# Algy/fast-slic

Hardware: AMD Instinct MI355X
Metric: megapixels/sec @10 iters (1280x720 & 4K, K=1600); % HBM roofline (higher is better)
Workload: dtype u8/u16/i32 (integer SLIC); 1 GPU; 1280x720 RGB, K=1600, 10 iters (configs[1]), 8 frames/GPU; frames_per_gpu=8, global_frames=8, slots_per_gpu=6, submissions_per_launch_group=up to 2 (dynamic batching of the pipeline), inputs=device-resident uint8 RGB, device int16 labels, parallelism=frames sharded across GPUs, no collective

## Files before the change

### fast_slic_amd/csrc/assign.hip

```cpp
#include "device_common.h"
#include <type_traits>

namespace fslic {



template <int R, bool FUSE, bool LUT>
__global__ __launch_bounds__(256) void k_assign(FrameDev f, int rem, int stride, int Hv, int buf, int sbuf) {
    extern __shared__ uint32_t s_lut[];
    __shared__ uint32_t s_rawbuf[kWavesPerBlock][3 * 64];
    __shared__ uint4 s_listbuf[kWavesPerBlock][64];
    __shared__ uint32_t s_accbuf[FUSE ? kWavesPerBlock * kAccSlots * 6 * kAccCopies : 1];

    f.select(blockIdx.z);
    const uint32_t gen = f.generation();
    const int tid = threadIdx.x;
    const int lane = tid & 63;
    const int wave = (int)rfl((uint32_t)(tid >> 6));
    uint32_t* const s_raw = s_rawbuf[wave];
    uint4* const s_list = s_listbuf[wave];
    uint32_t* const s_acc = s_accbuf + (FUSE ? wave * (kAccSlots * 6 * kAccCopies) : 0);
    const int W = f.W, S = f.S;
    const int x0 = blockIdx.x * kTileW;
    const int x = x0 + lane;
// ... 118 lines not shown
        };
        for (int c0 = 0; c0 < total; c0 += 64) {
            const int e = c0 + lane;
            ClusterRec rec;
            rec.yx = 0; rec.lab = 0; rec.tag = 0; rec.pad = 0;
            if (e < total) rec = citems[cell_slot(e)];
            stream(rec, e < total && rec.pad == gen && in_window(rec, win));
        }
        for (uint32_t i0 = 0; i0 < novf; i0 += 64) {
            const uint32_t i = i0 + lane;
            ClusterRec rec;
            rec.yx = 0; rec.lab = 0; rec.tag = 0; rec.pad = 0;
            if (i < novf) rec = oitems[i];
            stream(rec, i < novf && in_window(rec, win));
        }
#pragma unroll
        for (int r = 0; r < R; ++r) {
            if (!(okx && r < nrows)) continue;
            const int y = yw_lo + r * stride;
            const size_t p = (size_t)y * W + x;
            uint32_t lbl;
            if (bw[r] < kHuge) { lbl = bt[r] & 0xFFFFu; f.labels[p] = (uint16_t)lbl; }
            else if (f.first_visit(y)) { lbl = 0xFFFFu; f.labels[p] = (uint16_t)0xFFFFu; }
            else lbl = f.labels[p];
            if (FUSE && lbl != 0xFFFFu) global_accumulate(f.sums[0], lbl, (uint32_t)y, (uint32_t)x, pix[r]);
        }
        return;
    }

    int n;
    {
        const bool act = lane < nraw;
        const uint32_t yx_j = act ? s_raw[lane] : 0u;
        const uint32_t lab_j = act ? s_raw[64 + lane] : 0u;
        const uint32_t tag_j = act ? s_raw[128 + lane] : 0xFFFFFFFFu;
        bool dup = false;
        for (int i = 0; i < nraw; ++i) {
            const uint32_t ty = __builtin_amdgcn_readlane(yx_j, i);
            const uint32_t tl = __builtin_amdgcn_readlane(lab_j, i);
            const uint32_t tt = __builtin_amdgcn_readlane(tag_j, i);
            dup = dup || (act && (tt < tag_j) && (ty == yx_j) && (tl == lab_j));
        }
        const unsigned long long dupmask = __ballot(dup);
        int rank = 0;
        for (int i = 0; i < nraw; ++i) {
            const uint32_t tt = __builtin_amdgcn_readlane(tag_j, i);
            rank += (int)((((dupmask >> i) & 1ull) == 0ull) && tt < tag_j);
        }
        if (act && !dup) s_list[rank] = make_uint4(yx_j, lab_j, tag_j & 0xFFFFu, 0u);
        n = nraw - __popcll(dupmask);
    }
    __builtin_amdgcn_wave_barrier();

    uint32_t best[R];
#pragma unroll
    for (int r = 0; r < R; ++r) best[r] = 0xFFFFFFFFu;
    uint2 nxt = *reinterpret_cast<const uint2*>(&s_list[0]);
#pragma unroll 1
    for (int c = 0; c < n; ++c) {
        const uint2 rec = nxt;
        nxt = *reinterpret_cast<const uint2*>(&s_list[min(c + 1, 63)]);
        const uint32_t cyx = rfl(rec.x);
        const uint32_t clab = rfl(rec.y);
        const int cy = (int)(cyx >> 16), cx = (int)(cyx & 0xFFFFu);
        const uint32_t A = spatial_A(cx);
#pragma unroll
        for (int r = 0; r < R; ++r) {
            const uint32_t w = dist_w(r, cy, clab, A);
            best[r] = min(best[r], LUT ? (w | (uint32_t)c) : ((w & hi16) | (uint32_t)c));
        }
    }

    uint32_t slot[R];
#pragma unroll
    for (int r = 0; r < R; ++r) {
        const int y = yw_lo + r * stride;
        const bool ok = okx && r < nrows;
        const bool found = best[r] < kHuge;
        const uint32_t idx = found ? (best[r] & 0xFFFFu) : 0u;
        const uint32_t k = s_list[idx].z;
        slot[r] = 0xFFFFFFFFu;
        if (ok) {
            const size_t p = (size_t)y * W + x;
            if (found) {
                f.labels[p] = (uint16_t)k;
                if (FUSE) {
                    if (idx < (uint32_t)kAccSlots) slot[r] = idx;
                    else global_accumulate(f.sums[0], k, (uint32_t)y, (uint32_t)x, pix[r]);
                }
            } else if (f.first_visit(y)) {
                f.labels[p] = (uint16_t)0xFFFFu;
            } else if (FUSE) {
                const uint32_t old = f.labels[p];
                if (old != 0xFFFFu) global_accumulate(f.sums[0], old, (uint32_t)y, (uint32_t)x, pix[r]);
            }
        }
    }
    if (FUSE) {
        bool uni = slot[0] != 0xFFFFFFFFu;
#pragma unroll
        for (int r = 1; r < R; ++r) uni = uni && (slot[r] == slot[0]);
        const uint32_t copy = (uint32_t)lane & (kAccCopies - 1);
        if (uni) {
            uint32_t sL = 0, sa = 0, sb = 0;
#pragma unroll
            for (int r = 0; r < R; ++r) { sL += pix[r] & 255u; sa += (pix[r] >> 8) & 255u; sb += (pix[r] >> 16) & 255u; }
            uint32_t* a = s_acc + (slot[0] * 6) * kAccCopies + copy;
            atomicAdd(a + 0 * kAccCopies, (uint32_t)R);
            atomicAdd(a + 1 * kAccCopies, (uint32_t)(R * yw_lo + stride * (R * (R - 1) / 2)));
            atomicAdd(a + 2 * kAccCopies, (uint32_t)(R * x));
            atomicAdd(a + 3 * kAccCopies, sL);
            atomicAdd(a + 4 * kAccCopies, sa);
            atomicAdd(a + 5 * kAccCopies, sb);
        } else {
#pragma unroll
            for (int r = 0; r < R; ++r) {
                if (slot[r] != 0xFFFFFFFFu) {
                    uint32_t* a = s_acc + (slot[r] * 6) * kAccCopies + copy;
                    atomicAdd(a + 0 * kAccCopies, 1u);
                    atomicAdd(a + 1 * kAccCopies, (uint32_t)(yw_lo + r * stride));
                    atomicAdd(a + 2 * kAccCopies, (uint32_t)x);
                    atomicAdd(a + 3 * kAccCopies, pix[r] & 255u);
                    atomicAdd(a + 4 * kAccCopies, (pix[r] >> 8) & 255u);
                    atomicAdd(a + 5 * kAccCopies, (pix[r] >> 16) & 255u);
                }
            }
        }
        __builtin_amdgcn_wave_barrier();
        const int nacc = min(n, kAccSlots) * 6;
        for (int i = lane; i < nacc; i += 64) {
            uint32_t v = 0;
#pragma unroll
            for (int c = 0; c < kAccCopies; ++c) v += s_acc[i * kAccCopies + c];
            if (v) {
                const int sl = i / 6;
                atomicAdd(f.sums[0] + 6 * (size_t)s_list[sl].z + (i - sl * 6), v);
            }
        }
    }
}

typedef unsigned short us2 __attribute__((ext_vector_type(2)));

constexpr uint32_t kNoSlot = 0xFFFFFFFFu;
constexpr int kRawBuffer = 0x00020000;
constexpr int kAuxSc1 = 16;

static __device__ __forceinline__ us2 key_pair(uint32_t dist01, uint32_t idx01) {
    uint32_t r;
    asm("v_pk_mad_u16 %0, %1, 64, %2 op_sel_hi:[1,0,1] clamp" : "=v"(r) : "v"(dist01), "s"(idx01));
    return __builtin_bit_cast(us2, r);
}


static __device__ __forceinline__ unsigned long long sbitrep(uint32_t v) {
    unsigned long long r;
    asm("s_bitreplicate_b64_b32 %0, %1" : "=s"(r) : "s"(v));
    return r;
}
static __device__ __forceinline__ void min_in_place(us2& best, us2 key) {
    uint32_t b = __builtin_bit_cast(uint32_t, best);
    asm("v_pk_min_u16 %0, %0, %1" : "+v"(b) : "v"(__builtin_bit_cast(uint32_t, key)));
    best = __builtin_bit_cast(us2, b);
}

template <int R>
static __device__ __forceinline__ void row_masks(uint32_t inv, uint32_t (&m)[R / 2]) {
    static_assert(R == 8 || R == 16 || R == 32, "row masks are built for 8, 16 or 32 rows");
    if constexpr (R == 32) {
        uint32_t lo[8], hi[8];
        row_masks<16>(inv & 0xFFFFu, lo);
        row_masks<16>(inv >> 16, hi);
#pragma unroll
        for (int q = 0; q < 8; ++q) { m[q] = lo[q]; m[8 + q] = hi[q]; }
        return;
    }
    const unsigned long long r1 = sbitrep(inv);
    const unsigned long long r2 = sbitrep((uint32_t)r1);
    if (R == 8) {
        const unsigned long long r3 = sbitrep((uint32_t)r2);
        const unsigned long long a = sbitrep((uint32_t)r3), b = sbitrep((uint32_t)(r3 >> 32));
        m[0] = (uint32_t)a; m[1] = (uint32_t)(a >> 32); m[2] = (uint32_t)b; m[3] = (uint32_t)(b >> 32);
    } else {
        const unsigned long long r3a = sbitrep((uint32_t)r2), r3b = sbitrep((uint32_t)(r2 >> 32));
        const unsigned long long q0 = sbitrep((uint32_t)r3a), q1 = sbitrep((uint32_t)(r3a >> 32));
        const unsigned long long q2 = sbitrep((uint32_t)r3b), q3 = sbitrep((uint32_t)(r3b >> 32));
        m[0] = (uint32_t)q0; m[1] = (uint32_t)(q0 >> 32); m[2] = (uint32_t)q1; m[3] = (uint32_t)(q1 >> 32);
        m[R / 2 - 4] = (uint32_t)q2; m[R / 2 - 3] = (uint32_t)(q2 >> 32); m[R / 2 - 2] = (uint32_t)q3; m[R / 2 - 1] = (uint32_t)(q3 >> 32);
    }
}

#if defined(FSLIC_LAB) && FSLIC_LAB == 4
#define ASG_STAMP(i_, cond_) do { if ((cond_) && lane == 0) { asm volatile("" ::: "memory"); asg_w[(i_)] = (uint32_t)__builtin_amdgcn_s_memrealtime() - asg_t0; asm volatile("" ::: "memory"); } } while (0)
#define ASG_PUT(i_, cond_, v_) do { if ((cond_) && lane == 0) asg_w[(i_)] = (uint32_t)(v_); } while (0)
#else
#define ASG_STAMP(i_, cond_) do { } while (0)
#define ASG_PUT(i_, cond_, v_) do { } while (0)
#endif
#ifdef FSLIC_MARKS
#define ASG_MARK(name_) asm volatile("; @@MARK " name_ ::: "memory")
#else
#define ASG_MARK(name_) do { } while (0)
#endif
static __device__ __forceinline__ void lds_dma_16(const void* gsrc, uint32_t lds_byte_addr) {
    uint32_t keep;
    asm volatile("s_mov_b32 %0, m0\n\ts_mov_b32 m0, %2\n\ts_nop 0\n\tglobal_load_lds_dwordx4 %1, off\n\ts_mov_b32 m0, %0"
                 : "=&s"(keep) : "v"(gsrc), "s"(lds_byte_addr) : "memory");
}

static __device__ __forceinline__ uint32_t ld_agent(const uint32_t* p) { return __hip_atomic_load(p, __ATOMIC_RELAXED, __HIP_MEMORY_SCOPE_AGENT); }
static __device__ __forceinline__ unsigned long long ld_agent64(const void* p) {
    return __hip_atomic_load(reinterpret_cast<const unsigned long long*>(p), __ATOMIC_RELAXED, __HIP_MEMORY_SCOPE_AGENT);
}
static __device__ __forceinline__ void bin_insert_next(const FrameDev& f, uint32_t k, uint32_t yx, uint32_t lab) {
    const int y = (int)(yx >> 16), x = (int)(yx & 0xFFFFu);
    const uint32_t phase = 2u * (div_by((uint32_t)y, (uint32_t)f.T, f.T_rcp) & 1u) + (div_by((uint32_t)x, (uint32_t)f.T, f.T_rcp) & 1u);
    ClusterRec rec;
    rec.yx = yx; rec.lab = lab; rec.tag = (phase << 16) | k; rec.pad = f.generation() + 1u;
    f.cl_tag[k] = rec.tag;
    const int cell = (y >> f.cs_shift) * f.ncx + (x >> f.cs_shift);
    const uint32_t slot = atomicAdd(&f.cell_cnt[1][cell], 1u);
    if (slot < (uint32_t)kCellCap) f.cell_items[1][(size_t)cell * kCellCap + slot] = rec;
    else f.ovf_items[1][atomicAdd(f.ovf_cnt[1], 1u)] = rec;
}
static __device__ __forceinline__ void fused_finalize(const FrameDev& f, uint32_t k, uint32_t yx, uint32_t lab, uint32_t nx, uint32_t ny, uint32_t b0, uint32_t ymask) {
    uint32_t* const s0 = f.sums[0] + 6 * (size_t)k;
    uint32_t s[6];
#pragma unroll
    for (int q = 0; q < 6; ++q) s[q] = ld_agent(s0 + q);
    const char* const cp = reinterpret_cast<const char*>(f.cpart + (size_t)k * f.cpart_ns * 6);
    const uint32_t ne = nx * ny;
    const uint32_t inv_nx = (uint32_t)(65536.0f * __builtin_amdgcn_rcpf((float)nx)) + 1u;
    constexpr int kBatch = 4;
    for (uint32_t e0 = 0; e0 < ne; e0 += kBatch) {
        unsigned long long v[kBatch][3];
#pragma unroll
        for (int u = 0; u < kBatch; ++u) {
            const uint32_t e = e0 + (uint32_t)u;
            uint32_t ey = __umul24(e, inv_nx) >> 16;
            if (__umul24(ey, nx) > e) ey--;
            const uint32_t ex = e - __umul24(ey, nx);
            v[u][0] = v[u][1] = v[u][2] = 0ull;
            if (e < ne) {
                const char* p = cp + __umul24(cpart_slot((b0 >> 16) + ey, (b0 & 0xFFFFu) + ex, ymask, (uint32_t)f.nbx), 24u);
                v[u][0] = ld_agent64(p); v[u][1] = ld_agent64(p + 8); v[u][2] = ld_agent64(p + 16);
            }
        }
#pragma unroll
        for (int u = 0; u < kBatch; ++u) {
            s[0] += (uint32_t)v[u][0]; s[1] += (uint32_t)(v[u][0] >> 32); s[2] += (uint32_t)v[u][1]; s[3] += (uint32_t)(v[u][1] >> 32);
            s[4] += (uint32_t)v[u][2]; s[5] += (uint32_t)(v[u][2] >> 32);
        }
    }
    const uint32_t n = s[0];
    f.cl_n[k] = n;
    if (n != 0) {
        const uint32_t h = n >> 1, r = 0xFFFFFFFFu / n;
        int y = (int)div_by(s[1] + h, n, r), x = (int)div_by(s[2] + h, n, r);
        y = min(max(y, 0), f.H - 1);
        x = min(max(x, 0), f.W - 1);
        const uint32_t L = div_by(s[3] + h, n, r), a = div_by(s[4] + h, n, r), b = div_by(s[5] + h, n, r);
        yx = ((uint32_t)y << 16) | (uint32_t)x;
        lab = (L & 255u) | ((a & 255u) << 8) | ((b & 255u) << 16);
        f.cl_lab[k] = lab;
        f.cl_moved[k] = 1;
        f.cl_yx[k] = yx;
    }
#pragma unroll
    for (int q = 0; q < 6; ++q) s0[q] = 0u;
    f.cl_arrive[k] = 0u;
    bin_insert_next(f, k, yx, lab);
    if (n != 0 && k + 1u < (uint32_t)f.K && f.cl_shadow[k + 1u]) {
        f.cl_shadow[k + 1u] = 0u;
        bin_insert_next(f, k + 1u, f.cl_yx[k + 1u], f.cl_lab[k + 1u]);
    }
}

struct BlkMap { uint32_t gx, gy; };
static inline BlkMap blk_map(dim3 g) { BlkMap m; m.gx = g.x; m.gy = g.y; return m; }
static inline dim3 blk_grid(dim3 g) { return dim3(g.x, g.z, g.y); }

template <int R, bool FUSE, int STRIDE, bool VT, bool FBIN = false, bool PRE = false>
static __device__ __forceinline__ void assign_blk2_body(FrameDev& f, int rem, int Hv, const BlkMap& bm) {
    static_assert(!FBIN || FUSE, "the cluster pass rides on the fused centroid sums");
    static_assert(!PRE || (FUSE && !FBIN), "preemptive mode: the fused pass with its own flush");
    const uint32_t bxi = blockIdx.x, byi = blockIdx.z, bzi = blockIdx.y;
    extern __shared__ __attribute__((aligned(16))) uint32_t s_dyn[];
    __shared__ __attribute__((aligned(16))) uint4 s_raw[kWavesPerBlock][64];
    __shared__ __attribute__((aligned(16))) uint32_t s_part[64][4];
    __shared__ __attribute__((aligned(16))) uint32_t s_wcnt[4];
    __shared__ __attribute__((aligned(16))) uint32_t s_entry[FUSE ? 64 : 4];
    __shared__ __attribute__((aligned(16))) uint16_t s_klab[64];
    __shared__ __attribute__((aligned(16))) unsigned long long s_acc[FUSE ? 64 * kBlkCopies * 2 : 2];
    static_assert(R % 2 == 0, "rows are processed in pairs");
    constexpr int BH = kWavesPerBlock * R;
    static_assert(!FUSE || (BH * 64 * 255 < (1 << 20) && (BH - 1) * STRIDE * BH * 64 < (1 << 20)), "accumulator fields overflow");

    ASG_MARK("entry");
    f.select((int)bzi);
    const uint32_t gen = f.generation();
    const int tid = threadIdx.x;
    if (FBIN) {

        const uint32_t gi = (byi * bm.gx + bxi) * 256u + (uint32_t)tid;
        if (gi < (uint32_t)f.ncell) f.cell_cnt[0][gi] = 0u;
        if (gi == 0u) *f.ovf_cnt[2] = 0u;
// ... 182 lines not shown
        uint32_t va_j, vb_j;
        {
            const int dy0 = yw_lo - (int)(yx_j >> 16);
            const int rs = min(max(div_stride(-dy0 + STRIDE * BIAS + STRIDE - 1) - BIAS, 0), R);
            const int ra = min(max(div_stride(-S - dy0 + STRIDE * BIAS + STRIDE - 1) - BIAS, 0), R);
            const int rb = min(max(div_stride(S - dy0 + STRIDE * BIAS) - BIAS, -1), R - 1);
            const uint32_t upto_rs = low_bits(rs);
            const uint32_t in_win = rb < 0 ? 0u : (low_bits(rb + 1) & ~low_bits(ra) & full);
            va_j = in_win & upto_rs;
            vb_j = in_win & ~upto_rs;
        }
        const uint4* const s_rv = reinterpret_cast<const uint4*>(s_dyn);
        auto pass = [&](uint32_t clab, uint32_t base, uint32_t idx01, const uint32_t* mq) {
            uint32_t spw[R / 2];
            {
                const uint4 e0 = s_rv[base];
                spw[0] = e0.x; spw[1] = e0.y; spw[2] = e0.z; spw[3] = e0.w;
#pragma unroll
                for (int h = 1; h < R / 8; ++h) {
                    const uint4 e1 = s_rv[base + 8 * h * STRIDE];
                    spw[4 * h] = e1.x; spw[4 * h + 1] = e1.y; spw[4 * h + 2] = e1.z; spw[4 * h + 3] = e1.w;
                }
            }
            uint32_t t[R / 2];
#pragma unroll
            for (int q = 0; q < R / 2; ++q) {
                const uint32_t s0 = __builtin_amdgcn_sad_u8(pix[2 * q], clab, spw[q]);
                t[q] = __builtin_amdgcn_sad_hi_u8(pix[2 * q + 1], clab, s0);
            }
            us2 key[R / 2];
#pragma unroll
            for (int q = 0; q < R / 2; ++q) key[q] = key_pair(t[q], mq ? (mq[q] | idx01) : idx01);
#pragma unroll
            for (int q = 0; q < R / 2; ++q) min_in_place(best[q], key[q]);
        };
        unsigned long long todo_wa = todo & ballot(va_j == full);
        unsigned long long todo_wb = todo & ballot(vb_j == full);
        unsigned long long todo_above = todo & ballot(va_j != 0u) & ~todo_wa;
        unsigned long long todo_below = todo & ballot(vb_j != 0u) & ~todo_wb;
        auto fetch = [&](int c, uint32_t& clab, uint32_t& uxc, uint32_t& k0, uint32_t& idx01, auto clamp_tag) {
            constexpr bool CLAMP = decltype(clamp_tag)::value;
            const uint32_t cyx = __builtin_amdgcn_readlane(yx_j, c);
            const uint32_t clabx = __builtin_amdgcn_readlane(lab_j, c);
            clab = clabx & 0x00FFFFFFu;
            const int cy = (int)(cyx >> 16), cx = (int)(cyx & 0xFFFFu);
            const uint32_t ux = __builtin_amdgcn_sad_u16((uint32_t)x, (uint32_t)cx, 0u);
            uxc = CLAMP ? (ux <= (uint32_t)S ? ux : xout) : ux;
            k0 = (uint32_t)(Cc + yw_lo - cy);
            idx01 = (clabx >> 24) * 0x10001u;
        };
#pragma unroll 1
        while (todo_wa) {
            const int c = __builtin_ctzll(todo_wa);
            todo_wa &= todo_wa - 1ull;
            uint32_t clab, uxc, k0, idx01;
            fetch(c, clab, uxc, k0, idx01, std::false_type{});
            if (uxc <= (uint32_t)S) pass(clab, k0 - uxc, idx01, nullptr);
        }
#pragma unroll 1
        while (todo_wb) {
            const int c = __builtin_ctzll(todo_wb);
            todo_wb &= todo_wb - 1ull;
            uint32_t clab, uxc, k0, idx01;
            fetch(c, clab, uxc, k0, idx01, std::false_type{});
            if (uxc <= (uint32_t)S) pass(clab, k0 + uxc, idx01, nullptr);
        }
        if constexpr (R == 16 && FUSE) {
            auto pass_half = [&](auto half_tag, uint32_t clab, uint32_t base, uint32_t idx01, const uint32_t* mq4) {
                constexpr int HF = decltype(half_tag)::value;
                const uint4 e0 = s_rv[base + 8 * HF * STRIDE];
                const uint32_t spw[4] = {e0.x, e0.y, e0.z, e0.w};
                uint32_t t[4];
#pragma unroll
                for (int q = 0; q < 4; ++q) {
                    const uint32_t s0 = __builtin_amdgcn_sad_u8(pix[2 * (4 * HF + q)], clab, spw[q]);
                    t[q] = __builtin_amdgcn_sad_hi_u8(pix[2 * (4 * HF + q) + 1], clab, s0);
                }
                us2 key[4];
#pragma unroll
                for (int q = 0; q < 4; ++q) key[q] = key_pair(t[q], mq4[q] | idx01);
#pragma unroll
                for (int q = 0; q < 4; ++q) min_in_place(best[4 * HF + q], key[q]);
            };
            auto masked = [&](unsigned long long m, const uint32_t rows_j, auto sign_tag) {
                constexpr int SG = decltype(sign_tag)::value;
                unsigned long long m_lo = m & ballot((rows_j & 0xFF00u) == 0u);
                unsigned long long m_hi = m & ballot((rows_j & 0x00FFu) == 0u) & ~m_lo;
                unsigned long long m_both = m & ~m_lo & ~m_hi;
#pragma unroll 1
                while (m_lo) {
                    const int c = __builtin_ctzll(m_lo);
                    m_lo &= m_lo - 1ull;
                    uint32_t clab, uxc, k0, idx01, mq[4];
                    fetch(c, clab, uxc, k0, idx01, std::true_type{});
                    row_masks<8>(~__builtin_amdgcn_readlane(rows_j, c) & 0xFFu, mq);
                    pass_half(std::integral_constant<int, 0>{}, clab, SG < 0 ? k0 - uxc : k0 + uxc, idx01, mq);
                }
#pragma unroll 1
                while (m_hi) {
                    const int c = __builtin_ctzll(m_hi);
                    m_hi &= m_hi - 1ull;
                    uint32_t clab, uxc, k0, idx01, mq[4];
                    fetch(c, clab, uxc, k0, idx01, std::true_type{});
                    row_masks<8>(~(__builtin_amdgcn_readlane(rows_j, c) >> 8) & 0xFFu, mq);
                    pass_half(std::integral_constant<int, 1>{}, clab, SG < 0 ? k0 - uxc : k0 + uxc, idx01, mq);
                }
#pragma unroll 1
                while (m_both) {
                    const int c = __builtin_ctzll(m_both);
                    m_both &= m_both - 1ull;
                    uint32_t clab, uxc, k0, idx01, mq[R / 2];
                    fetch(c, clab, uxc, k0, idx01, std::true_type{});
                    row_masks<R>(~__builtin_amdgcn_readlane(rows_j, c) & full, mq);
                    pass(clab, SG < 0 ? k0 - uxc : k0 + uxc, idx01, mq);
                }
            };
            masked(todo_above, va_j, std::integral_constant<int, -1>{});
            masked(todo_below, vb_j, std::integral_constant<int, 1>{});
        } else {
#pragma unroll 1
            while (todo_above) {
                const int c = __builtin_ctzll(todo_above);
                todo_above &= todo_above - 1ull;
                uint32_t clab, uxc, k0, idx01, mq[R / 2];
                fetch(c, clab, uxc, k0, idx01, std::true_type{});
                row_masks<R>(~__builtin_amdgcn_readlane(va_j, c) & full, mq);
                pass(clab, k0 - uxc, idx01, mq);
            }
#pragma unroll 1
            while (todo_below) {
                const int c = __builtin_ctzll(todo_below);
                todo_below &= todo_below - 1ull;
                uint32_t clab, uxc, k0, idx01, mq[R / 2];
                fetch(c, clab, uxc, k0, idx01, std::true_type{});
                row_masks<R>(~__builtin_amdgcn_readlane(vb_j, c) & full, mq);
                pass(clab, k0 + uxc, idx01, mq);
            }
        }
    } else {
        constexpr int HQ = R / 4;
        static_assert(R % 4 == 0, "two halves of whole row pairs");
        unsigned long long todo_b, todo_u, todo_l;
        {
            const int cyj = (int)(yx_j >> 16);
            const int yh = yw_lo + (R / 2) * STRIDE;
            const unsigned long long up = todo & ballot(cyj <= yw_lo + (R / 2 - 1) * STRIDE + S);
            const unsigned long long lo = todo & ballot(cyj >= yh - S) & ballot(cyj <= yh + (R / 2 - 1) * STRIDE + S);
            todo_b = up & lo;
            todo_u = up & ~lo;
            todo_l = lo & ~up;
        }
        uint32_t pitch_v;
        asm volatile("v_mov_b32 %0, %1" : "=v"(pitch_v) : "s"(nrpad * 4u));
        const char* const tab_b = reinterpret_cast<const char*>(s_dyn);
        auto walk = [&](unsigned long long m, auto q0_tag, auto nq_tag) {
            constexpr int Q0 = decltype(q0_tag)::value, NQ = decltype(nq_tag)::value;
#pragma unroll 1
            while (m) {
                const int c = __builtin_ctzll(m);
                m &= m - 1ull;
                const uint32_t cyx = __builtin_amdgcn_readlane(yx_j, c);
                const uint32_t clabx = __builtin_amdgcn_readlane(lab_j, c);
                const uint32_t clab = clabx & 0x00FFFFFFu;
                const int cy = (int)(cyx >> 16), cx = (int)(cyx & 0xFFFFu);
                const uint32_t ux = __builtin_amdgcn_sad_u16((uint32_t)x, (uint32_t)cx, 0u);
                const uint32_t uxc = min(ux, (uint32_t)(S + 1));
                const uint32_t a0 = __umul24(uxc, pitch_v) + (uint32_t)(yw_lo - cy + dyoff) * 4u;
                const uint32_t idx01 = (clabx >> 24) * 0x10001u;
                uint32_t t[NQ];
#pragma unroll
                for (int q = 0; q < NQ; ++q) {
                    const uint32_t sp = *reinterpret_cast<const uint32_t*>(tab_b + a0 + (uint32_t)((2 * (Q0 + q)) * STRIDE * 4));
                    const uint32_t s0 = __builtin_amdgcn_sad_u8(pix[2 * (Q0 + q)], clab, sp);
                    t[q] = __builtin_amdgcn_sad_hi_u8(pix[2 * (Q0 + q) + 1], clab, s0);
                }
                us2 key[NQ];
#pragma unroll
                for (int q = 0; q < NQ; ++q) key[q] = key_pair(t[q], idx01);
#pragma unroll
                for (int q = 0; q < NQ; ++q) min_in_place(best[Q0 + q], key[q]);
            }
        };
        if constexpr (R == 16 && FUSE) {
            (void)todo_b; (void)todo_u; (void)todo_l;
            unsigned long long cov[4];
            {
                const int cyj = (int)(yx_j >> 16);
#pragma unroll
                for (int q = 0; q < 4; ++q) {
                    const int ylo = yw_lo + q * (R / 4) * STRIDE, yhi = ylo + (R / 4 - 1) * STRIDE;
                    cov[q] = todo & ballot(cyj >= ylo - S) & ballot(cyj <= yhi + S);
                }
            }
            constexpr int P = R / 8;
            auto quarters = [&](unsigned long long m, auto q0, auto nq) {
                walk(m, std::integral_constant<int, decltype(q0)::value * P>{}, std::integral_constant<int, decltype(nq)::value * P>{});
            };
            using I0 = std::integral_constant<int, 0>; using I1 = std::integral_constant<int, 1>; using I2 = std::integral_constant<int, 2>;
            using I3 = std::integral_constant<int, 3>; using I4 = std::integral_constant<int, 4>;
            quarters(cov[0] & cov[3], I0{}, I4{});
            quarters(cov[0] & cov[2] & ~cov[3], I0{}, I3{});
            quarters(cov[1] & cov[3] & ~cov[0], I1{}, I3{});
            quarters(cov[0] & cov[1] & ~cov[2], I0{}, I2{});
            quarters(cov[1] & cov[2] & ~cov[0] & ~cov[3], I1{}, I2{});
            quarters(cov[2] & cov[3] & ~cov[1], I2{}, I2{});
            quarters(cov[0] & ~cov[1], I0{}, I1{});
            quarters(cov[1] & ~cov[0] & ~cov[2], I1{}, I1{});
            quarters(cov[2] & ~cov[1] & ~cov[3], I2{}, I1{});
            quarters(cov[3] & ~cov[2], I3{}, I1{});
        } else {
            walk(todo_b, std::integral_constant<int, 0>{}, std::integral_constant<int, 2 * HQ>{});
            walk(todo_u, std::integral_constant<int, 0>{}, std::integral_constant<int, HQ>{});
            walk(todo_l, std::integral_constant<int, HQ>{}, std::integral_constant<int, HQ>{});
        }
    }

    ASG_MARK("after_walk");
    ASG_STAMP(4, wave == 0);
    ASG_PUT(9, wave == 0, __popcll(todo));
    ASG_PUT(10, wave == 0, bn);
    __builtin_amdgcn_s_waitcnt(0x0F70);
    bool epilogue_done = false;
    {
        us2 worst = best[0];
#pragma unroll
        for (int q = 1; q < R / 2; ++q) worst = __builtin_elementwise_max(worst, best[q]);
        const bool all_found = (ballot(worst.x == 0xFFFF) | ballot(worst.y == 0xFFFF)) == 0ull;
        bool fast_ok = all_found && nrows == R;
        if constexpr (PRE) fast_ok = fast_ok && rfl(f.pre_flags[0]) != 0u;
        if (fast_ok) {
            ASG_MARK("labels");
            epilogue_done = true;
            if (okx) {
                uint32_t kk[R];
                const char* const ktab = reinterpret_cast<const char*>(s_klab);
#pragma unroll
                for (int q = 0; q < R / 2; ++q) {
                    const uint32_t b = __builtin_bit_cast(uint32_t, best[q]) & 0x003F003Fu;
                    kk[2 * q] = *reinterpret_cast<const uint16_t*>(ktab + ((b & 0xFFu) << 1));
                    kk[2 * q + 1] = *reinterpret_cast<const uint16_t*>(ktab + (((b >> 16) & 0xFFu) << 1));
                }
                const __amdgpu_buffer_rsrc_t ws = __builtin_amdgcn_make_buffer_rsrc(f.labels, 0, (int)((uint32_t)f.N * 2u), kRawBuffer);
                const uint32_t so0 = (uint32_t)yw_lo * (uint32_t)W * 2u, pitch2 = (uint32_t)(STRIDE * W) * 2u;
#pragma unroll
                for (int r = 0; r < R; ++r)
                    __builtin_amdgcn_raw_buffer_store_b16((uint16_t)kk[r], ws, (int)((uint32_t)x * 2u), (int)(so0 + (uint32_t)r * pitch2), kAuxSc1);
                ASG_STAMP(5, wave == 0);
                ASG_MARK("sums");
                if (FUSE) {
                    const uint32_t copy16 = ((uint32_t)lane & (kBlkCopies - 1)) * 16u;
                    const uint32_t dyw = (uint32_t)(wave * R * STRIDE);
                    char* const accb = reinterpret_cast<char*>(s_acc);
                    uint32_t sL = 0, sa = 0, sb = 0;
                    uint32_t wq[R / 2];
#pragma unroll
                    for (int q = 0; q < R / 2; ++q) wq[q] = __builtin_bit_cast(uint32_t, best[q]) & 0x003F003Fu;
                    auto words = [&](int cnt, unsigned long long& A, unsigned long long& B) {
                        const uint32_t a_lo = sL | (sa << 20), a_hi = (sa >> 12) | (sb << 8);
                        const uint32_t ys = (uint32_t)cnt * dyw + (uint32_t)(STRIDE * (cnt * (cnt - 1) / 2));
                        const uint32_t b_lo = __umul24((uint32_t)lane, (uint32_t)cnt) + (ys << 20), b_hi = (uint32_t)cnt << 8;
                        A = (unsigned long long)a_lo | ((unsigned long long)a_hi << 32);
                        B = (unsigned long long)b_lo | ((unsigned long long)b_hi << 32);
                    };
                    unsigned long long prevA = 0ull, prevB = 0ull;
#pragma unroll
                    for (int r = 0; r < R; ++r) {
                        const uint32_t p = pix[r];
                        sL = __builtin_amdgcn_udot4(p, 0x00000001u, sL, false);
                        sa = __builtin_amdgcn_udot4(p, 0x00000100u, sa, false);
                        sb = __builtin_amdgcn_udot4(p, 0x00010000u, sb, false);
                        if (r == R - 1) break;
                        const uint32_t cur = (r & 1) ? (wq[r / 2] >> 16) : (wq[r / 2] & 0xFFFFu);
                        const uint32_t nxt = (r & 1) ? (wq[r / 2 + 1] & 0xFFFFu) : (wq[r / 2] >> 16);
#if FSLIC_EXP & 1
                        if (false) {
#else
                        if (cur != nxt) {
#endif
                            unsigned long long A, B;
                            words(r + 1, A, B);
                            unsigned long long* const run = reinterpret_cast<unsigned long long*>(accb + (cur * (uint32_t)(kBlkCopies * 16) + copy16));
                            atomicAdd(run, A - prevA);
                            atomicAdd(run + 1, B - prevB);
                            prevA = A; prevB = B;
                        }
                    }
                    {
                        unsigned long long A, B;
                        words(R, A, B);
                        unsigned long long* const last = reinterpret_cast<unsigned long long*>(accb + ((wq[R / 2 - 1] >> 16) * (uint32_t)(kBlkCopies * 16) + copy16));
                        atomicAdd(last, A - prevA);
                        atomicAdd(last + 1, B - prevB);
                    }
                }
            }
        }
    }
    ASG_MARK("slow_epilogue");
    if (!epilogue_done) {
        uint32_t slot[R];
        uint16_t* rowp = f.labels + (size_t)yw_lo * W;
        const uint32_t xo = (uint32_t)x;
#pragma unroll
        for (int r = 0; r < R; ++r) {
            const bool ok = okx && r < nrows;
            const uint32_t key = (r & 1) ? (uint32_t)best[r / 2].y : (uint32_t)best[r / 2].x;
            const bool found = key != 0xFFFFu;
            slot[r] = kNoSlot;
            if (ok && found) st_stream(rowp + xo, s_klab[key & 63u]);
            const bool unlabelled = !FBIN && ok && !found && (FUSE ? f.fv_mod == 1 : f.first_visit(yw_lo + r * STRIDE));
            if (unlabelled) st_stream(rowp + xo, (uint16_t)0xFFFFu);
            bool summed = FUSE && ok && !unlabelled;
            if constexpr (PRE) summed = summed && in_update(f, yw_lo + r * STRIDE, x);
            if (summed) {
                if (found) slot[r] = key & 63u;
                else {
                    const uint32_t old = rowp[xo];
                    if (old != 0xFFFFu) {
                        global_accumulate(f.sums[0], old, (uint32_t)(yw_lo + r * STRIDE), xo, pix[r]);
                        if (FBIN) atomicOr(f.err_flag, 2u);
                    }
                }
            }
            rowp += (size_t)STRIDE * W;
        }
        ASG_STAMP(5, wave == 0);
        if (FUSE) {
            const uint32_t copy = (uint32_t)lane & (kBlkCopies - 1);
            const uint32_t dyw = (uint32_t)(wave * R * STRIDE);
            uint32_t cur = slot[0], a_lo = 0, a_hi = 0, b_lo = 0, b_hi = 0;
            auto flush = [&]() {
                if (cur != kNoSlot) {
                    unsigned long long* a = s_acc + (cur * kBlkCopies + copy) * 2;
// ... 289 lines not shown
```

Baseline: 64100 megapixels/sec.

## Pair left-zone and right-zone centers into one lane-divergent candidate pass

```diff
diff --git a/fast_slic_amd/csrc/assign.hip b/fast_slic_amd/csrc/assign.hip
--- a/fast_slic_amd/csrc/assign.hip
+++ b/fast_slic_amd/csrc/assign.hip
@@ -294,6 +294,14 @@
     return __builtin_bit_cast(us2, r);
 }
 
+
+static __device__ __forceinline__ us2 key_pair_v(uint32_t dist01, uint32_t idx01) {
+    uint32_t r;
+    asm("v_pk_mad_u16 %0, %1, 64, %2 op_sel_hi:[1,0,1] clamp" : "=v"(r) : "v"(dist01), "v"(idx01));
+    return __builtin_bit_cast(us2, r);
+}
+template <int R, bool FUSE>
+constexpr bool kPairWalk = R == 16;
 
 static __device__ __forceinline__ unsigned long long sbitrep(uint32_t v) {
     unsigned long long r;
@@ -782,33 +790,75 @@
         }
         uint32_t pitch_v;
         asm volatile("v_mov_b32 %0, %1" : "=v"(pitch_v) : "s"(nrpad * 4u));
-        const char* const tab_b = reinterpret_cast<const char*>(s_dyn);
+        typedef const __attribute__((address_space(3))) uint32_t* lds_word_ptr;
+        const uint32_t tab_b = (uint32_t)(size_t)(__attribute__((address_space(3))) uint32_t*)s_dyn;
+        constexpr bool PAIR = kPairWalk<R, FUSE>;
+        unsigned long long zone_l = 0ull, zone_r = 0ull;
+        if constexpr (PAIR) {
+            const int cxj = (int)(yx_j & 0xFFFFu);
+            zone_l = ballot(cxj <= x0 + 31 - S);
+            zone_r = ballot(cxj >= x0 + 32 + S);
+        }
         auto walk = [&](unsigned long long m, auto q0_tag, auto nq_tag) {
             constexpr int Q0 = decltype(q0_tag)::value, NQ = decltype(nq_tag)::value;
+            auto rows = [&](uint32_t a0, uint32_t clab, uint32_t idx01, auto vec_tag) {
+                uint32_t t[NQ];
+#pragma unroll
+                for (int q = 0; q < NQ; ++q) {
+                    const uint32_t sp = *(lds_word_ptr)(size_t)(a0 + (uint32_t)((2 * (Q0 + q)) * STRIDE * 4));
+                    const uint32_t s0 = __builtin_amdgcn_sad_u8(pix[2 * (Q0 + q)], clab, sp);
+                    t[q] = __builtin_amdgcn_sad_hi_u8(pix[2 * (Q0 + q) + 1], clab, s0);
+                }
+                us2 key[NQ];
+#pragma unroll
+                for (int q = 0; q < NQ; ++q) {
+                    if constexpr (decltype(vec_tag)::value) key[q] = key_pair_v(t[q], idx01);
+                    else key[q] = key_pair(t[q], idx01);
+                }
+#pragma unroll
+                for (int q = 0; q < NQ; ++q) min_in_place(best[Q0 + q], key[q]);
+            };
+            unsigned long long single = m;
+            if constexpr (PAIR) {
+                unsigned long long ml = m & zone_l, mr = m & zone_r;
 #pragma unroll 1
-            while (m) {
-                const int c = __builtin_ctzll(m);
-                m &= m - 1ull;
+                while ((ml != 0ull) & (mr != 0ull)) {
+                    const int c = __builtin_ctzll(ml), p = __builtin_ctzll(mr);
+                    ml &= ml - 1ull;
+                    mr &= mr - 1ull;
+                    const uint32_t cyx = __builtin_amdgcn_readlane(yx_j, c), pyx = __builtin_amdgcn_readlane(yx_j, p);
+                    const uint32_t clabx_c = __builtin_amdgcn_readlane(lab_j, c), clabx_p = __builtin_amdgcn_readlane(lab_j, p);
+                    const uint32_t ux_c = __builtin_amdgcn_sad_u16((uint32_t)x, cyx & 0xFFFFu, 0u);
+                    const uint32_t ux_p = __builtin_amdgcn_sad_u16((uint32_t)x, pyx & 0xFFFFu, 0u);
+                    uint32_t other = ux_p < ux_c ? 0xFFFFFFFFu : 0u;
+                    asm("" : "+v"(other));
+                    const uint32_t uxc = min(min(ux_c, ux_p), (uint32_t)(S + 1));
+                    const uint32_t row_c = tab_b + (uint32_t)(yw_lo - (int)(cyx >> 16) + dyoff) * 4u;
+                    int back = ((int)(pyx >> 16) - (int)(cyx >> 16)) * 4;
+                    asm("" : "+s"(back));
+                    uint32_t a0 = __umul24(uxc, pitch_v) + row_c;
+                    asm("v_mad_i32_i24 %0, %1, %2, %0" : "+v"(a0) : "v"(other), "s"(back));
+                    uint32_t dlab = clabx_c ^ clabx_p;
+                    asm("" : "+s"(dlab));
+                    uint32_t tlab = other & dlab;
+                    asm("" : "+v"(tlab));
+                    uint32_t clabx = clabx_c ^ tlab;
+                    asm("" : "+v"(clabx));
+                    rows(a0, clabx & 0x00FFFFFFu, __builtin_amdgcn_perm(clabx, clabx, 0x0C030C03u), std::true_type{});
+                }
+                single = (m & ~(zone_l | zone_r)) | ml | mr;
+            }
+#pragma unroll 1
+            while (single) {
+                const int c = __builtin_ctzll(single);
+                single &= single - 1ull;
                 const uint32_t cyx = __builtin_amdgcn_readlane(yx_j, c);
                 const uint32_t clabx = __builtin_amdgcn_readlane(lab_j, c);
-                const uint32_t clab = clabx & 0x00FFFFFFu;
                 const int cy = (int)(cyx >> 16), cx = (int)(cyx & 0xFFFFu);
                 const uint32_t ux = __builtin_amdgcn_sad_u16((uint32_t)x, (uint32_t)cx, 0u);
                 const uint32_t uxc = min(ux, (uint32_t)(S + 1));
-                const uint32_t a0 = __umul24(uxc, pitch_v) + (uint32_t)(yw_lo - cy + dyoff) * 4u;
-                const uint32_t idx01 = (clabx >> 24) * 0x10001u;
-                uint32_t t[NQ];
-#pragma unroll
-                for (int q = 0; q < NQ; ++q) {
-                    const uint32_t sp = *reinterpret_cast<const uint32_t*>(tab_b + a0 + (uint32_t)((2 * (Q0 + q)) * STRIDE * 4));
-                    const uint32_t s0 = __builtin_amdgcn_sad_u8(pix[2 * (Q0 + q)], clab, sp);
-                    t[q] = __builtin_amdgcn_sad_hi_u8(pix[2 * (Q0 + q) + 1], clab, s0);
-                }
-                us2 key[NQ];
-#pragma unroll
-                for (int q = 0; q < NQ; ++q) key[q] = key_pair(t[q], idx01);
-#pragma unroll
-                for (int q = 0; q < NQ; ++q) min_in_place(best[Q0 + q], key[q]);
+                const uint32_t a0 = __umul24(uxc, pitch_v) + (tab_b + (uint32_t)(yw_lo - cy + dyoff) * 4u);
+                rows(a0, clabx & 0x00FFFFFFu, (clabx >> 24) * 0x10001u, std::false_type{});
             }
         };
         if constexpr (R == 16 && FUSE) {
```

After: 64020 megapixels/sec. Within noise of the previous version (-0.1%).
